# HarryL-Git/ampnet

Hardware: AMD Instinct MI355X
Metric: AMPConv edges/sec (fwd+bwd) (higher is better)
Workload: dtype f32

## Files before the change

### ampnet_amd/_lib.py

```python
import ctypes
import os

import torch

_HERE = os.path.dirname(os.path.abspath(__file__))
LIB_PATH = os.environ.get('AMPCONV_LIB_PATH', os.path.join(_HERE, 'libampconv.so'))

EXPECTED_ABI = 111

AMPCONV_F32 = 0
AMPCONV_BF16 = 1
DTYPES = {torch.float32: AMPCONV_F32, torch.bfloat16: AMPCONV_BF16}
PASS_FWD, PASS_DST, PASS_SRC = 0, 1, 2
FAMILY_BF16_MFMA, FAMILY_SMALL, FAMILY_MFMA, FAMILY_BLOCK, FAMILY_GENERIC = range(5)
HUB_CHUNK = int(os.environ.get('AMPCONV_HUB_CHUNK', 0))


def hub_chunk(num_edges):
    return HUB_CHUNK if HUB_CHUNK > 0 else (128 if num_edges >= (1 << 20) else 64)
COLSUM_BLOCKS = 1024


class View(ctypes.Structure):
    _fields_ = [('ptr', ctypes.c_void_p), ('node_stride', ctypes.c_int64),
# ... 90 lines not shown
    'ampconv_absmax': (_i32, [_vp, _i64, _i64, _i32, _i32, _vp, _i32, _vp]),
    'ampconv_planes_supported': (_i32, [_i32, _i32, _i32]),
    'ampconv_fwd_edge_planes': (_i32, [View, View, View, _vp, _vp, _i64, _i32, _i32, _i32, View, _vp, _i64, _vp, _vp, _vp]),
    'ampconv_bwd_edge_dst_planes': (_i32, [View, View, View, View, _vp, _vp, _i64, _i32, _i32, _i32, View, _vp, _i64, _vp,
                                           _vp, _vp, _vp, _vp, _vp]),
    'ampconv_bwd_edge_src_planes': (_i32, [View, View, View, View, _vp, _vp, _i64, _i32, _i32, _i32, View, View, _vp, _i64,
                                           _vp, _vp, _vp, _vp, _vp]),
    'ampconv_scaled_supported': (_i32, [_i32, _i32, _i32]),
    'ampconv_fwd_edge_scaled': (_i32, [View, View, View, _vp, _vp, _i64, _i32, _i32, _i32, View, _vp, _i64, _vp, _vp, _vp]),
    'ampconv_bwd_edge_dst_scaled': (_i32, [View, View, View, View, _vp, _vp, _i64, _i32, _i32, _i32, View, _vp, _i64, _vp,
                                           _vp, _vp, _vp, _vp, _vp]),
    'ampconv_bwd_edge_src_scaled': (_i32, [View, View, View, View, _vp, _vp, _vp, _i64, _i32, _i32, _i32, View, View, _vp,
                                           _i64, _vp, _vp, _vp, _vp, _vp]),
    'ampconv_token_supported': (_i32, [_i32, _i32, _i32, _i32]),
    'ampconv_fwd_edge_token': (_i32, [View, View, View, _vp, _vp, _i64, _i32, _i32, _i32, View, _vp, _i64, _vp, _i32, _vp]),
    'ampconv_bwd_edge_dst_token': (_i32, [View, View, View, View, _vp, _vp, _i64, _i32, _i32, _i32, View, _vp, _i64, _vp,
                                          _i32, _vp]),
    'ampconv_bwd_edge_src_token': (_i32, [View, View, View, View, _vp, _vp, _vp, _i64, _i32, _i32, _i32, View, View, _vp,
                                          _i64, _vp, _i32, _vp]),
    'ampconv_proj_out_bound': (_i32, [_vp, _i64, _i64, _i32, _i32, _vp, _vp, _vp, _vp]),
    'ampconv_proj_rows_planes': (_i32, [_vp, _i64, _i64, _i32, _vp, _i32, _vp, _vp, _i32, _i32, _vp, _i64, _vp, _vp, _vp,
                                        _i32, _i32, _vp]),
    'ampconv_planes_to_f32': (_i32, [_vp, _i64, _i64, _i32, _i32, _vp, _vp, _i64, _vp]),
    'ampconv_absmax_stats': (_i32, [_vp, _i64, _i64, _i32, _vp, _vp]),
    'ampconv_active_nodes_workspace_bytes': (_sz, [_i64]),
    'ampconv_active_nodes': (_i32, [_vp, _vp, _i64, _i32, _vp, _vp, _vp, _vp, _sz, _vp]),
    'ampconv_segment_mean': (_i32, [_vp, _vp, _vp, _i64, _i64, _vp, _vp]),
    'ampconv_mask_rows': (_i32, [_vp, _vp, _i64, _i64, _i32, _vp]),
    'ampconv_masked_colsum': (_i32, [_vp, _vp, _i64, _i32, _i32, _vp, _i32, _vp]),
    'ampconv_act_dropout_fwd': (_i32, [_vp, _i64, _i32, ctypes.c_uint64, ctypes.c_uint32, ctypes.c_float, _vp, _i32, _vp]),
    'ampconv_act_dropout_bwd': (_i32, [_vp, _vp, _i64, _i32, ctypes.c_uint64, ctypes.c_uint32, ctypes.c_float, _vp, _i32, _vp]),
    'ampconv_pool_fwd': (_i32, [_vp, _i64, _i32, _i32, _i32, _i32, ctypes.c_uint64, ctypes.c_uint32, ctypes.c_float, _vp, _i32,
                                _vp]),
    'ampconv_pool_bwd': (_i32, [_vp, _vp, _i64, _i32, _i32, _i32, _i32, ctypes.c_uint64, ctypes.c_uint32, ctypes.c_float, _vp,
                                _i32, _vp]),
    'ampconv_head_workspace_bytes': (_sz, [_i64, _i32, _i32]),
    'ampconv_head_fwd': (_i32, [_vp, _i64, _i32, _i64, _vp, _vp, _i32, _i32, _vp, _i32, _vp]),
    'ampconv_head_bwd': (_i32, [_vp, _i64, _i32, _i64, _vp, _i32, _i32, _vp, _vp, _vp, _vp, _vp, _vp, _sz, _i32, _vp]),
    'ampconv_head_nll_fwd': (_i32, [_vp, _i64, _i32, _i64, _vp, _vp, _i32, _vp, _vp, _vp, _i32, _i32, _vp, _vp, _vp, _vp,
                                    _i32, _vp]),
    'ampconv_head_nll_bwd': (_i32, [_vp, _i64, _i32, _i64, _vp, _vp, _i32, _vp, _vp, _vp, _i32, _i32, _vp, _vp, _vp, _vp,
                                    _vp, _sz, _i32, _vp]),
    'ampconv_norm_workspace_bytes': (_sz, [_i64, _i32]),
    'ampconv_norm_fwd': (_i32, [_vp, _i64, _i32, _vp, _vp, ctypes.c_float, _i32, ctypes.c_uint64, ctypes.c_uint32,
                                ctypes.c_float, _vp, _vp, _i32, _vp]),
    'ampconv_norm_bwd': (_i32, [_vp, _vp, _vp, _i64, _i32, _vp, _vp, _i32, ctypes.c_uint64, ctypes.c_uint32, ctypes.c_float,
# ... 75 lines not shown
```

### ampnet_amd/conv/functional.py

```python
import dataclasses
import os

import torch

from .. import _lib
from .._lib import ptr as _ptr
from ..graph import EdgeCSR, _stream
from .projection import (Projections, _aligned, _tn_matmul, gemm_precision, mask_rows, masked_colsum,
                         proj_image, proj_images, proj_native, proj_rows, proj_wgrad)


def _view(buf2d, col_off, L, dh):
    assert buf2d.is_contiguous() and buf2d.dtype in (torch.float32, torch.bfloat16)
    W = buf2d.size(1)
    return _lib.View(buf2d.data_ptr() + buf2d.element_size() * col_off, L * W, W, dh)


SOFTMAX_STATS = os.environ.get('AMPCONV_SOFTMAX_STATS', '1') != '0'
NODE_LISTS = os.environ.get('AMPCONV_NODE_LISTS', '1') != '0'
PROJ_SCALED = os.environ.get('AMPCONV_PROJ_SCALED', '1') != '0'
PROJ_SCALED_MIN_ELEMENTS = 1 << 24


EDGE_PLANES = os.environ.get('AMPCONV_EDGE_PLANES', '1') != '0'
# ... 8 lines not shown
        if (hit is not None and hit[0]() is key and hit[1] == key._version and hit[4] == (key.data_ptr(), tuple(key.shape))
                and hit[2].device == t2.device):
            return hit[2], hit[3]
    lib = _lib.load()
    t2 = _aligned(t2)
    st = torch.empty(2, dtype=torch.float32, device=t2.device)
    _lib.check(lib.ampconv_absmax_stats(t2.data_ptr(), t2.stride(0), t2.size(0), t2.size(1), st.data_ptr(), _stream()),
               'ampconv_absmax_stats')
    amax, smin = st.tolist()
    narrow = not (smin * float(1 << RANGE_LOG2) < amax)
    if key is not None:
        if len(_STATS_CACHE) >= 16:
            for k in [k for k, v in _STATS_CACHE.items() if v[0]() is None] or list(_STATS_CACHE)[:8]:
                _STATS_CACHE.pop(k, None)
        _STATS_CACHE[id(key)] = (weakref.ref(key), key._version, st, narrow, (key.data_ptr(), tuple(key.shape)))
    return st, narrow


def planes_to_f32(buf2d, bound, dh=32):
    out = torch.empty_like(buf2d)
    _lib.check(_lib.load().ampconv_planes_to_f32(buf2d.data_ptr(), buf2d.stride(0), buf2d.size(0), buf2d.size(1), dh,
                                                 bound.data_ptr(), out.data_ptr(), out.stride(0), _stream()),
               'ampconv_planes_to_f32')
    return out


def proj_out_bound(W, transpose, bias, amax, out):
    R, C = W.shape
    N, K = (C, R) if transpose else (R, C)
    sn, sk = (1, W.stride(0)) if transpose else (W.stride(0), 1)
    _lib.check(_lib.load().ampconv_proj_out_bound(W.data_ptr(), sn, sk, N, K, _ptr(bias), amax.data_ptr(), out.data_ptr(),
                                                  _stream()), 'ampconv_proj_out_bound')


def proj_rows_planes(a2, image, bound, bias=None, rowptr=None, L=0, row_scale=0, amax=None, out_amax=None, amax_col0=0,
                     dh=32):
    lib = _lib.load()
    img, N, K, wdt = image
    assert a2.dim() == 2 and a2.size(1) == K and a2.stride(1) == 1 and a2.dtype == wdt == torch.float32
    a2 = _aligned(a2)
    out = torch.empty(a2.size(0), N, dtype=wdt, device=a2.device)
    _lib.check(lib.ampconv_proj_rows_planes(a2.data_ptr(), a2.stride(0), a2.size(0), K, img.data_ptr(), N, _ptr(bias),
                                            _ptr(rowptr), L, row_scale, out.data_ptr(), out.stride(0), amax.data_ptr(),
                                            bound.data_ptr(), _ptr(out_amax), amax_col0, dh, _stream()),
               'ampconv_proj_rows_planes')
    return out
# ... 401 lines not shown
```

### ampnet_amd/csrc/edge_block_x3.hip

```cpp
#include "plane16.h"

namespace {
using namespace plane16;

constexpr int kRowB = 128;
constexpr int kTileRowsB = 16 * kRowB;

#define MFMA_X3(a, b, c) \
  __builtin_amdgcn_mfma_f32_16x16x32_bf16(__builtin_bit_cast(bf16x8, a), __builtin_bit_cast(bf16x8, b), (c), 0, 0, 0)
#define MFMA_XH(a, b, c) \
  __builtin_amdgcn_mfma_f32_16x16x32_f16(__builtin_bit_cast(f16x8, a), __builtin_bit_cast(f16x8, b), (c), 0, 0, 0)

template <int P>
struct XFrag {
  i32x4 p[P];
};

__device__ __forceinline__ float bfl(int u) { return __builtin_bit_cast(float, u << 16); }
__device__ __forceinline__ float bfh(int u) { return __builtin_bit_cast(float, u & (int)0xFFFF0000u); }

__device__ __forceinline__ int xoff(int j, int ch) { return j * kRowB + ((ch ^ (((j >> 1) & 3) << 1)) << 4); }

struct XArgs {
  ampconv_view_t Q, K, V, dO, O, dK, dV;
// ... 458 lines not shown
  __device__ __forceinline__ float dk_mul(const XArgs &a) const { return part_or(a, a.oscale); }
  __device__ __forceinline__ float dv_mul() const { return 1.f; }
};

template <int KS>
__device__ __forceinline__ float own_max_norm2(const XFrag<2> (&f)[KS]) {
  float q = frag_sumsq(f[0].p[0]);
  if constexpr (KS == 2) q += frag_sumsq(f[1].p[0]);
  const float t = groups_sum(q);
  return __builtin_bit_cast(float, __builtin_amdgcn_readfirstlane(__builtin_bit_cast(int, row16_max(t))));
}
__device__ __forceinline__ float ds_scale_x(float own2, float other) {
  return plane_scale(2.f * __builtin_sqrtf(own2) * (8.f * other));
}

struct FmtXH : Fp32Storage {
  static constexpr int kPlanes = 2;
  using Frag = XFrag<2>;
  static constexpr bool kQidx = false, kRecordMax = true, kSrcPairs = AMPCONV_XH_SRC_PAIRS;
  static constexpr float kPScale = 16384.f, kPUnscale = 1.f / 16384.f;
  static constexpr int fwd_mcb(int) { return AMPCONV_XH_FWD_MCB; }
  static constexpr int dst_mcb(int) { return AMPCONV_XH_DST_MCB; }

  static __device__ __forceinline__ void split(float x0, float x1, int (&w)[2]) { split2(x0, x1, w[0], w[1]); }
  static __device__ __forceinline__ f32x4 mma(const Frag &a, const Frag &b, f32x4 c) {
    c = MFMA_XH(a.p[1], b.p[0], c);
    c = MFMA_XH(a.p[0], b.p[1], c);
    return MFMA_XH(a.p[0], b.p[0], c);
  }

  float sq, uq, sg, ug;
  float sc;
  float sd, usd;
  __device__ __forceinline__ FmtXH(const XArgs &a, bool grad)
      : sq(plane_scale(a.bounds[0])), uq(1.f / sq), sg(grad ? plane_scale(a.bounds[1]) : 1.f), ug(1.f / sg),
        sc((a.qscale * uq) * uq), sd(1.f), usd(1.f) {}
  __device__ __forceinline__ float q_mul(const XArgs &) const { return sq; }
  __device__ __forceinline__ float g_mul(float inv) const { return inv * sg; }
  __device__ __forceinline__ float kv_mul() const { return sq; }
  template <int KS>
  __device__ __forceinline__ void dst_own(const Frag (&gf)[KS], const XArgs &a) {
    sd = ds_scale_x(own_max_norm2(gf), a.bounds[2] * sq);
    usd = 1.f / sd;
  }
  template <int KS>
  __device__ __forceinline__ void src_own(const Frag (&vf)[KS], const XArgs &a) {
    sd = ds_scale_x(own_max_norm2(vf), a.bounds[3] * sg);
// ... 627 lines not shown
```

### ampnet_amd/csrc/edge_mfma_bf16.hip

```cpp
#include "edge_wave16.h"

namespace {
using namespace wave16;

typedef unsigned short bf16_t;


#define MFMA_BF16(a, b, c) \
  __builtin_amdgcn_mfma_f32_16x16x32_bf16(__builtin_bit_cast(bf16x8, a), __builtin_bit_cast(bf16x8, b), (c), 0, 0, 0)

struct Args {
  ampconv_view_t Q, K, V, dO, O, dK, dV;
  const int32_t *ptr, *idx, *qidx;
  const float *cinv;
  HubArgs hub;
  int64_t n_units;
  int L, H;
  float qscale, oscale;
};

template <bool HALF>
__device__ __forceinline__ void store_tile(const ampconv_view_t &v, int64_t node, int h, const f32x4 (&T)[2][2],
                                           float scale, bool to_f32, int L, int lane) {
  const int g = lane >> 4;
// ... 4 lines not shown
#pragma unroll
      for (int mc = 0; mc < (HALF ? 1 : 2); ++mc) {
        const float a = T[mc][nt][0] * scale, b = T[mc][nt][1] * scale, c = T[mc][nt][2] * scale,
                    d = T[mc][nt][3] * scale;
        const int64_t off = node * v.node_stride + (int64_t)h * v.head_stride + (int64_t)i * v.row_stride +
                            4 * g + 16 * mc;
        if (to_f32)
          *reinterpret_cast<float4 *>(reinterpret_cast<float *>(v.ptr) + off) = make_float4(a, b, c, d);
        else
          *reinterpret_cast<i32x2 *>(reinterpret_cast<bf16_t *>(v.ptr) + off) =
              i32x2{cvt_pk_bf16(a, b), cvt_pk_bf16(c, d)};
      }
    }
  }
}

struct FmtB {
  using Args = ::Args;
  static constexpr int kPlanes = 1, kElemBytes = 2, kLoOff = 0, kTileBytes = kPlaneBytes;
  using Frag = wave16::Frag<1>;
  template <bool HALF> using Geom = PairGeom<4, 3, HALF ? 2 : 4, 1>;
  static constexpr bool kHalfZeroLds = false;
  template <bool HALF> static constexpr int mc_tiles() { return 2; }
  static constexpr bool kShadow = false;
  static constexpr float kMasked = kNegBig, kPMul = 1.f;

  static __device__ __forceinline__ f32x4 mma(const Frag &a, const Frag &b, f32x4 c) { return MFMA_BF16(a.p[0], b.p[0], c); }
  static __device__ __forceinline__ Frag cd_frag(const f32x4 &t0, const f32x4 &t1) {
    return Frag{{i32x4{cvt_pk_bf16(t0[0], t0[1]), cvt_pk_bf16(t0[2], t0[3]), cvt_pk_bf16(t1[0], t1[1]),
                       cvt_pk_bf16(t1[2], t1[3])}}};
  }

  struct Scales {
    float sc;
  };
  template <bool HALF> static __device__ __forceinline__ Scales scales(const Args &a) { return Scales{a.qscale}; }
  static __device__ __forceinline__ int64_t qrow(const Args &a, int64_t r) { return a.qidx ? uniform_ld(a.qidx + r) : r; }
  static __device__ __forceinline__ float fwd_scale(const Scales &, float mean) { return mean; }
  static __device__ __forceinline__ float ds_mul(const Args &, int deg, const Frag (&)[2]) {
    return deg > 0 ? 1.f / (float)deg : 0.f;
  }
  template <bool HALF> static __device__ __forceinline__ float dq_scale(const Args &a, const Scales &, float, bool hubp) {
    return hubp ? 1.f : a.oscale;
  }

  template <bool HALF>
  static __device__ __forceinline__ float store(const ampconv_view_t &v, int64_t node, int h, const f32x4 (&T)[2][2],
// ... 195 lines not shown
```

### ampnet_amd/csrc/edge_mfma_f16x2.hip

```cpp
#include "edge_wave16.h"

namespace {
using namespace wave16;

constexpr int kLoOff = kPlaneBytes + 64;
constexpr int kTileBytes = kLoOff + kPlaneBytes;
constexpr float kPScale = 16384.f;
constexpr float kPUnscale = 1.f / 16384.f;
constexpr float kSqrtDh = 5.656854249492381f;
constexpr float kMasked = -__builtin_inff();

#define MFMA_F16(a, b, c) \
  __builtin_amdgcn_mfma_f32_16x16x32_f16(__builtin_bit_cast(f16x8, a), __builtin_bit_cast(f16x8, b), (c), 0, 0, 0)

__device__ __forceinline__ f32x4 mfma3(const i32x4 &ah, const i32x4 &al, const i32x4 &bh, const i32x4 &bl, f32x4 c) {
  c = MFMA_F16(al, bh, c);
  c = MFMA_F16(ah, bl, c);
  return MFMA_F16(ah, bh, c);
}

__device__ __forceinline__ float tile_max_norm2(const i32x4 &f0, const i32x4 &f1) {
  const float t = fmaxf(groups_sum(frag_sumsq(f0)), groups_sum(frag_sumsq(f1)));
  return __builtin_bit_cast(float, __builtin_amdgcn_readfirstlane(__builtin_bit_cast(int, row16_max(t))));
}
__device__ __forceinline__ float ds_scale(float own2, float other) {
  return plane_scale(2.f * __builtin_sqrtf(own2) * (kSqrtDh * other));
}

__device__ __forceinline__ void cd_frag2(const f32x4 &t0, float t1_0, i32x4 &hi, i32x4 &lo) {
  int h0, l0, h1, l1, h2, l2;
  split2(t0[0], t0[1], h0, l0);
  split2(t0[2], t0[3], h1, l1);
  split2(t1_0, 0.f, h2, l2);
  hi = i32x4{h0, h1, h2, 0};
  lo = i32x4{l0, l1, l2, 0};
}

struct Args {
  ampconv_view_t Q, K, V, dO, O, dK, dV;
  const int32_t *ptr, *idx;
  const float *bounds;
  float *absmax;
  const int32_t *spos;
  float *stats;
  HubArgs hub;
  int64_t n_units;
  int L, H;
};

template <bool QUARTER, int MC>
__device__ __forceinline__ float store_tile(const ampconv_view_t &v, int64_t node, int h, const f32x4 (&T)[MC][2],
                                            float scale, int L, int lane) {
  const int g = lane >> 4, n = lane & 15;
  float m = 0.f;
#pragma unroll
// ... 7 lines not shown
        const int64_t off = node * v.node_stride + (int64_t)h * v.head_stride + (int64_t)i * v.row_stride + 4 * g + 16 * mc;
        *reinterpret_cast<float4 *>(reinterpret_cast<float *>(v.ptr) + off) = o;
        m = finite_abs_max(m, o);
      }
    }
  }
  return m;
}

struct FmtP {
  using Args = ::Args;
  static constexpr int kPlanes = 2, kElemBytes = 4, kLoOff = ::kLoOff, kTileBytes = ::kTileBytes;
  using Frag = wave16::Frag<2>;
  template <bool HALF> using Geom = PairGeom<HALF ? 4 : 8, HALF ? 3 : 5, HALF ? 4 : 8, 2, ::kLoOff>;
  static constexpr bool kHalfZeroLds = true;
  template <bool HALF> static constexpr int mc_tiles() { return HALF ? 1 : 2; }
  static constexpr bool kShadow = true;
  static constexpr float kMasked = ::kMasked, kPMul = kPScale;

  static __device__ __forceinline__ f32x4 mma(const Frag &a, const Frag &b, f32x4 c) { return mfma3(a.p[0], a.p[1], b.p[0], b.p[1], c); }
  static __device__ __forceinline__ Frag cd_frag(const f32x4 &t0, const f32x4 &t1) {
    Frag f;
    cd_frag2(t0, t1[0], f.p[0], f.p[1]);
    return f;
  }

  struct Scales {
    float uq, ug, sc;
  };
  template <bool HALF> static constexpr float inv_sqrt_dh() { return HALF ? 0.25f : 0.17677669529663687f; }
  template <bool HALF> static __device__ __forceinline__ Scales scales(const Args &a) {
    const float uq = 1.f / plane_scale(uniform_ld(a.bounds)), ug = 1.f / plane_scale(uniform_ld(a.bounds + 1));
    return Scales{uq, ug, (kLog2e * inv_sqrt_dh<HALF>() * uq) * uq};
  }
  static __device__ __forceinline__ int64_t qrow(const Args &, int64_t r) { return r; }
  static __device__ __forceinline__ float fwd_scale(const Scales &k, float mean) { return kPUnscale * k.uq * mean; }
  static __device__ __forceinline__ float ds_mul(const Args &a, int, const Frag (&gB)[2]) {
    return ds_scale(tile_max_norm2(gB[0].p[0], gB[1].p[0]), uniform_ld(a.bounds + 2) * plane_scale(uniform_ld(a.bounds)));
  }
  template <bool HALF> static __device__ __forceinline__ float dq_scale(const Args &, const Scales &k, float ss, bool hubp) {
    return (((1.f / ss) * k.uq) * k.ug) * k.uq * (hubp ? 1.f : inv_sqrt_dh<HALF>());
  }

  template <bool HALF>
  static __device__ __forceinline__ float store(const ampconv_view_t &v, int64_t node, int h, const f32x4 (&T)[HALF ? 1 : 2][2],
                                                float scale, bool, int L, int lane) {
// ... 261 lines not shown
```

### ampnet_amd/csrc/edge_wave16.h

```cpp
#pragma once
#include "plane16.h"

namespace wave16 {
using namespace plane16;

constexpr int kWavesPerBlock = 4;
constexpr int DH = 32;
constexpr int kRowBytes = DH * 2;
constexpr int kPlaneBytes = kLmax * kRowBytes;

template <int P>
struct Frag {
  i32x4 p[P];
};

struct Unit {
  int lane, wave;
  int64_t row, onode;
  int h, beg, end, deg;
};
template <class Fmt, bool HALF, class Body>
__device__ __forceinline__ void for_unit(const typename Fmt::Args &a, const ampconv_view_t &out0, const ampconv_view_t *out1,
                                         const Body &body) {
  Unit u;
// ... 74 lines not shown
  for (int pl = 0; pl < P; ++pl) f.p[pl] = i32x4{0, 0, 0, 0};
  if (j < L && (!HALF || kg < 2)) {
#pragma unroll
    for (int pl = P - 1; pl >= 0; --pl)
      f.p[pl] = *reinterpret_cast<const i32x4 *>(base + (unsigned)j * row_bytes + pl * (HALF ? kRowBytes / 2 : kRowBytes) + 16 * kg);
  }
  return f;
}
template <class Fmt>
__device__ __forceinline__ typename Fmt::Frag lds_rowfrag(const char *img, int mt, int lane) {
  typename Fmt::Frag f;
#pragma unroll
  for (int pl = 0; pl < Fmt::kPlanes; ++pl) f.p[pl] = rowfrag(img + pl * Fmt::kLoOff, mt, lane);
  return f;
}
template <class Fmt>
__device__ __forceinline__ typename Fmt::Frag lds_colfrag(const char *img, int mc, int lane) {
  typename Fmt::Frag f;
#pragma unroll
  for (int pl = 0; pl < Fmt::kPlanes; ++pl) f.p[pl] = colfrag(img + pl * Fmt::kLoOff, mc, lane);
  return f;
}

template <bool FULL>
__device__ __forceinline__ float column_softmax(f32x4 &t0, f32x4 &t1, float sc, float mul, float masked, int L, int g) {
  if (!FULL) {
#pragma unroll
    for (int q = 0; q < 4; ++q)
      if (4 * g + q >= L) t0[q] = masked;
    if (16 + g >= L) t1[0] = masked;
  }
  float m = fmaxf(fmaxf(fmaxf(t0[0], t0[1]), fmaxf(t0[2], t0[3])), t1[0]);
  m = groups_max(m);
#pragma unroll
  for (int q = 0; q < 4; ++q) t0[q] = fast_exp2((t0[q] - m) * sc);
  t1[0] = fast_exp2((t1[0] - m) * sc);
  float l = ((t0[0] + t0[1]) + (t0[2] + t0[3])) + t1[0];
  l = groups_sum(l);
  const float inv = fast_rcp(l) * mul;
#pragma unroll
  for (int q = 0; q < 4; ++q) t0[q] *= inv;
  t1[0] *= inv;
  t1[1] = t1[2] = t1[3] = 0.f;
  return fmaf(m, sc, __builtin_amdgcn_logf(l));
}

template <class Fmt, bool FULL, bool HALF>
__device__ __forceinline__ void fwd_body(const typename Fmt::Args &a) {
  using F = typename Fmt::Frag;
  using G = typename Fmt::template Geom<HALF>;
  constexpr int MC = Fmt::template mc_tiles<HALF>(), TB = Fmt::kTileBytes, EB = Fmt::kElemBytes;
  __shared__ __attribute__((aligned(16))) char lds_all[kWavesPerBlock][2 * TB];
  for_unit<Fmt, HALF>(a, a.O, nullptr, [&](const Unit &u) __attribute__((always_inline)) {
    const int lane = u.lane, h = u.h, beg = u.beg, end = u.end;
    const int L = a.L, g = lane >> 4;
    char *Kt = lds_all[u.wave], *Vt = Kt + TB;
    const typename Fmt::Scales k = Fmt::template scales<HALF>(a);

    F qB[2];
    {
      const char *qb = slot_ptr<EB>(a.Q, Fmt::qrow(a, u.row), h);
      const unsigned rb = (unsigned)a.Q.row_stride * EB;
#pragma unroll
      for (int nt = 0; nt < 2; ++nt) qB[nt] = frag_global<Fmt::kPlanes, HALF, false>(qb, rb, nt, L, lane);
    }
    if (!FULL || (HALF && Fmt::kHalfZeroLds)) lds_zero(Kt, 2 * TB, lane);
    f32x4 OT[MC][2];
#pragma unroll
    for (int mc = 0; mc < MC; ++mc) OT[mc][0] = OT[mc][1] = f32x4{0.f, 0.f, 0.f, 0.f};

    Pair16<G::NLD> kv;
    IdxWindow win;
    const unsigned krb = (unsigned)a.K.row_stride * EB, vrb = (unsigned)a.V.row_stride * EB;
    auto fetch = [&](int p) {
      const int64_t s = idxwin_get<false>(win, a.idx, nullptr, p, end, lane, nullptr);
      pair16_load<FULL, G>(kv, slot_ptr<EB>(a.K, s, h), krb, slot_ptr<EB>(a.V, s, h), vrb, L, lane);
    };
    if (beg < end) {
      idxwin_load<false>(win, a.idx, nullptr, beg, end, lane);
      fetch(beg);
    }
    for (int p = beg; p < end; ++p) {
      pair16_to_lds<FULL, G, TB>(Kt, kv, L, lane);
      if (p + 1 < end) fetch(p + 1);
      __builtin_amdgcn_wave_barrier();

      f32x4 S[2][2];
#pragma unroll
      for (int mt = 0; mt < 2; ++mt) {
        const F kA = lds_rowfrag<Fmt>(Kt, mt, lane);
#pragma unroll
        for (int nt = 0; nt < 2; ++nt) S[mt][nt] = Fmt::mma(kA, qB[nt], f32x4{0.f, 0.f, 0.f, 0.f});
      }
      F pB[2];
#pragma unroll
      for (int nt = 0; nt < 2; ++nt) {
        column_softmax<FULL>(S[0][nt], S[1][nt], k.sc, Fmt::kPMul, Fmt::kMasked, L, g);
        if (!Fmt::kShadow) pB[nt] = Fmt::cd_frag(S[0][nt], S[1][nt]);
      }
      F vA[MC];
      if (Fmt::kShadow) TR_PRE_READ();
#pragma unroll
      for (int mc = 0; mc < MC; ++mc) vA[mc] = lds_colfrag<Fmt>(Vt, mc, lane);
      if (Fmt::kShadow) {
#pragma unroll
        for (int nt = 0; nt < 2; ++nt) pB[nt] = Fmt::cd_frag(S[0][nt], S[1][nt]);
      }
      TR_FRAG_FENCE();
#pragma unroll
      for (int mc = 0; mc < MC; ++mc)
#pragma unroll
        for (int nt = 0; nt < 2; ++nt) OT[mc][nt] = Fmt::mma(vA[mc], pB[nt], OT[mc][nt]);
      __builtin_amdgcn_wave_barrier();
    }
    const bool hubp = a.hub.mode == 2;
    Fmt::template store<HALF>(a.O, u.onode, h, OT, Fmt::fwd_scale(k, hubp ? 1.f : (u.deg > 0 ? 1.f / (float)u.deg : 0.f)),
                              hubp, L, lane);
  });
}

template <class Fmt, bool FULL, bool STATS, bool HALF>
__device__ __forceinline__ void bwd_dst_body(const typename Fmt::Args &a) {
  using F = typename Fmt::Frag;
  using G = typename Fmt::template Geom<HALF>;
  constexpr int MC = Fmt::template mc_tiles<HALF>(), TB = Fmt::kTileBytes, EB = Fmt::kElemBytes;
  __shared__ __attribute__((aligned(16))) char lds_all[kWavesPerBlock][2 * TB];
  for_unit<Fmt, HALF>(a, a.O, nullptr, [&](const Unit &u) __attribute__((always_inline)) {
    const int lane = u.lane, h = u.h, beg = u.beg, end = u.end;
    const int L = a.L, g = lane >> 4;
// ... 29 lines not shown
    if (beg < end) {
      idxwin_load<STATS>(win, a.idx, sposf, beg, end, lane);
      fetch(beg);
    }
    for (int p = beg; p < end; ++p) {
      pair16_to_lds<FULL, G, TB>(Kt, kv, L, lane);
      cposf = cposf_next;
      if (p + 1 < end) fetch(p + 1);
      __builtin_amdgcn_wave_barrier();

      f32x4 S[2][2], dP[2][2];
      float lse[2], dlt[2];
#pragma unroll
      for (int mt = 0; mt < 2; ++mt) {
        const F kA = lds_rowfrag<Fmt>(Kt, mt, lane);
        const F vA = lds_rowfrag<Fmt>(Vt, mt, lane);
#pragma unroll
        for (int nt = 0; nt < 2; ++nt) {
          S[mt][nt] = Fmt::mma(kA, qB[nt], f32x4{0.f, 0.f, 0.f, 0.f});
          dP[mt][nt] = Fmt::mma(vA, gB[nt], f32x4{0.f, 0.f, 0.f, 0.f});
        }
      }
      F sB[2];
#pragma unroll
      for (int nt = 0; nt < 2; ++nt) {
        lse[nt] = column_softmax<FULL>(S[0][nt], S[1][nt], k.sc, 1.f, Fmt::kMasked, L, g);
        float part = S[1][nt][0] * dP[1][nt][0];
#pragma unroll
        for (int q = 0; q < 4; ++q) part = fmaf(S[0][nt][q], dP[0][nt][q], part);
        const float delta = groups_sum(part);
        dlt[nt] = delta;
#pragma unroll
        for (int q = 0; q < 4; ++q) S[0][nt][q] *= (dP[0][nt][q] - delta) * dsm;
        S[1][nt][0] *= (dP[1][nt][0] - delta) * dsm;
        if (!Fmt::kShadow) sB[nt] = Fmt::cd_frag(S[0][nt], S[1][nt]);
      }
      F kC[MC];
      if (Fmt::kShadow) TR_PRE_READ();
#pragma unroll
      for (int mc = 0; mc < MC; ++mc) kC[mc] = lds_colfrag<Fmt>(Kt, mc, lane);
      if (Fmt::kShadow) {
#pragma unroll
        for (int nt = 0; nt < 2; ++nt) sB[nt] = Fmt::cd_frag(S[0][nt], S[1][nt]);
      }
      TR_FRAG_FENCE();
#pragma unroll
      for (int mc = 0; mc < MC; ++mc)
#pragma unroll
        for (int nt = 0; nt < 2; ++nt) dQT[mc][nt] = Fmt::mma(kC[mc], sB[nt], dQT[mc][nt]);
      if constexpr (STATS) {
        float *st = a.stats + ((int64_t)__builtin_bit_cast(int, cposf) * a.H + h) * kStatsPerUnit;
        if (lane < L) {
          st[lane] = lane < 16 ? lse[0] : lse[1];
          st[kLmax + lane] = lane < 16 ? dlt[0] : dlt[1];
        }
      }
      __builtin_amdgcn_wave_barrier();
    }
    const bool hubp = a.hub.mode == 2;
    const float m = Fmt::template store<HALF>(a.O, u.onode, h, dQT, Fmt::template dq_scale<HALF>(a, k, dsm, hubp), hubp, L, lane);
    Fmt::record_absmax(a, m);
  });
}

#define WAVE16_KERNELS(K) {{K<false, false>, K<true, false>}, {K<false, true>, K<true, true>}}
#define WAVE16_KERNELS_STATS(K, S) {{K<false, S, false>, K<true, S, false>}, {K<false, S, true>, K<true, S, true>}}
// ... 7 lines not shown
```

### ampnet_amd/csrc/operand_scale.hip

```cpp
#include "proj_common.h"

using namespace proj;

namespace {
__global__ __launch_bounds__(1024) void out_bound_kernel(const float *__restrict__ W, int64_t sn, int64_t sk, int N, int K,
                                                         const float *__restrict__ bias, const float *__restrict__ amax,
                                                         float *__restrict__ out) {
  __shared__ float red[2][16];
  const int lane = threadIdx.x & 63, w = threadIdx.x >> 6;
  float l1 = 0.f, bm = 0.f;
  for (int n = w; n < N; n += 16) {
    float sum = 0.f;
    for (int k = lane; k < K; k += 64) sum += finite_abs(W[(int64_t)n * sn + (int64_t)k * sk]);
    l1 = fmaxf(l1, wave_sum(sum));
  }
  if (bias)
    for (int n = threadIdx.x; n < N; n += 1024) bm = fmaxf(bm, finite_abs(bias[n]));
  bm = wave_max(bm);
  if (lane == 0) { red[0][w] = l1; red[1][w] = bm; }
  __syncthreads();
  if (threadIdx.x == 0) {
    for (int i = 1; i < 16; ++i) { l1 = fmaxf(l1, red[0][i]); bm = fmaxf(bm, red[1][i]); }
    out[0] = *amax * l1 + bm;
  }
// ... 31 lines not shown
    float *o = out + row * ldo + slot * dh + 8 * c;
    *reinterpret_cast<float4 *>(o) = make_float4(v[0], v[1], v[2], v[3]);
    *reinterpret_cast<float4 *>(o + 4) = make_float4(v[4], v[5], v[6], v[7]);
  }
}
}

extern "C" int ampconv_planes_to_f32(const void *X, int64_t ld, int64_t M, int K, int plane_dh, const float *bound, void *out,
                                     int64_t ldo, void *stream) {
  if (M < 0 || K <= 0 || (plane_dh != 32 && plane_dh != 16) || K % plane_dh || ld < K || ldo < K || ld % 4 || ldo % 4 || !bound)
    return AMPCONV_E_BADARG;
  if (M == 0) return AMPCONV_OK;
  if (!X || !out || (uintptr_t)X % 16 || (uintptr_t)out % 16) return AMPCONV_E_BADARG;
  const int64_t pieces = M * (K / 8);
  int64_t grid = (pieces + 255) / 256;
  const int64_t cap = (int64_t)cu_count() * 16;
  if (grid > cap) grid = cap;
  planes_to_f32_kernel<<<(unsigned)grid, 256, 0, (hipStream_t)stream>>>((const char *)X, ld, M, K / 8, plane_dh, bound,
                                                                        (float *)out, ldo);
  return ampconv_launch_status();
}

namespace {
template <typename T>
__global__ __launch_bounds__(256) void absmax_kernel(const T *__restrict__ X, int64_t ld, int64_t M, int K4,
                                                     float *__restrict__ out) {
  constexpr int EPP = 16 / sizeof(T);
  const int64_t total = M * K4;
  float m = 0.f;
  for (int64_t i = (int64_t)blockIdx.x * 256 + threadIdx.x; i < total; i += (int64_t)gridDim.x * 256) {
    const int64_t row = i / K4;
    const int c = (int)(i - row * K4);
    const uint4 raw = *reinterpret_cast<const uint4 *>(X + row * ld + (int64_t)c * EPP);
    if constexpr (sizeof(T) == 4) {
      m = fmaxf(m, fmaxf(fmaxf(finite_abs(__builtin_bit_cast(float, raw.x)), finite_abs(__builtin_bit_cast(float, raw.y))),
                         fmaxf(finite_abs(__builtin_bit_cast(float, raw.z)), finite_abs(__builtin_bit_cast(float, raw.w)))));
    } else {
      const unsigned u[4] = {raw.x, raw.y, raw.z, raw.w};
#pragma unroll
      for (int k = 0; k < 4; ++k)
        m = fmaxf(m, fmaxf(finite_abs(lo_as_f32(u[k])), finite_abs(hi_as_f32(u[k]))));
    }
  }
  __shared__ float red[4];
#pragma unroll
  for (int o = 32; o > 0; o >>= 1) m = fmaxf(m, __shfl_xor(m, o));
// ... 90 lines not shown
```

### ampnet_amd/csrc/plane16.h

```cpp
#pragma once
#include "mfma_tile.h"

namespace plane16 {

typedef int i32x4 __attribute__((ext_vector_type(4)));
typedef int i32x2 __attribute__((ext_vector_type(2)));
typedef float f32x2 __attribute__((ext_vector_type(2)));
typedef short s16x4 __attribute__((ext_vector_type(4)));
typedef _Float16 f16x2 __attribute__((ext_vector_type(2)));
typedef _Float16 f16x8 __attribute__((ext_vector_type(8)));
typedef __bf16 bf16x2 __attribute__((ext_vector_type(2)));
typedef __bf16 bf16x8 __attribute__((ext_vector_type(8)));

constexpr float kLog2e = 1.4426950408889634f;

__device__ __forceinline__ int cvt_pk_bf16(float a, float b) {
  f32x2 v = {a, b};
  return __builtin_bit_cast(int, __builtin_convertvector(v, bf16x2));
}
__device__ __forceinline__ int cvt_pk_f16(float a, float b) {
  f32x2 v = {a, b};
  return __builtin_bit_cast(int, __builtin_convertvector(v, f16x2));
}

__device__ __forceinline__ float plane_scale(float bound) {
  int e = (int)((__builtin_bit_cast(unsigned, bound) >> 23) & 0xFFu);
  e = e < 15 ? 15 : (e > 254 ? 254 : e);
  return __builtin_bit_cast(float, (unsigned)(268 - e) << 23);
}
__device__ __forceinline__ float plane_unscale(float bound) { return 1.f / plane_scale(bound); }

__device__ __forceinline__ void split2(float x0, float x1, int &h, int &l) {
  h = cvt_pk_f16(x0, x1);
  const f16x2 hv = __builtin_bit_cast(f16x2, h);
  l = cvt_pk_f16(x0 - (float)hv[0], x1 - (float)hv[1]);
}

__device__ __forceinline__ float frag_sumsq(const i32x4 &f) {
  float s = 0.f;
#pragma unroll
  for (int k = 0; k < 4; ++k) {
    const f16x2 v = __builtin_bit_cast(f16x2, f[k]);
    s = __builtin_amdgcn_fdot2(v, v, s, false);
  }
  return s;
}

__device__ __forceinline__ i32x2 tr_half(const char *p) {
  return __builtin_bit_cast(i32x2, __builtin_amdgcn_ds_read_tr16_b64_v4i16((__attribute__((address_space(3))) s16x4 *)p));
}
__device__ __forceinline__ i32x4 tr_frag(const char *p0, const char *p1) {
  const i32x2 ai = tr_half(p0), bi = tr_half(p1);
  return i32x4{ai[0], ai[1], bi[0], bi[1]};
}

// ... 38 lines not shown
```

### ampnet_amd/csrc/proj_gemm.hip

```cpp
#include <type_traits>
#include "proj_common.h"

namespace {
using namespace proj;

template <bool HP>
struct Pl {
  static constexpr int NP = HP ? 2 : 3;
  static constexpr int NQ = HP ? 3 : 6;
  static constexpr int kTile = NP * kFrag;
};
__device__ constexpr int kPA[2][6] = {{2, 1, 0, 1, 0, 0}, {1, 0, 0, 0, 0, 0}};
__device__ constexpr int kPB[2][6] = {{0, 1, 2, 0, 1, 0}, {0, 1, 0, 0, 0, 0}};
template <bool HP>
__device__ __forceinline__ f32x16 mfma_p(const i32x4 &a, const i32x4 &b, const f32x16 &c) {
  if constexpr (HP) return MFMA32H(a, b, c);
  else return MFMA32(a, b, c);
}

struct Pair3 {
  int h1, h2, h3;
};
__device__ __forceinline__ Pair3 split_pair(float x0, float x1) {
  const unsigned a = (unsigned)cvt_pk_bf16(x0, x1);
// ... 334 lines not shown
        const int ohi = a.plane_dh == 32 ? 16 * pc : 64 * (pc >> 1) + 16 * (pc & 1), olo = ohi + 2 * a.plane_dh;
#pragma unroll
        for (int i = 0; i < MTW; ++i) {
          const int rl0 = (MTW * wm + i) * 32;
          float fl[16];
#pragma unroll
          for (int g = 0; g < 4; ++g) {
            const float4 f4 = *reinterpret_cast<const float4 *>(fl_t + rl0 + 4 * fh + 8 * g);
            fl[4 * g] = f4.x; fl[4 * g + 1] = f4.y; fl[4 * g + 2] = f4.z; fl[4 * g + 3] = f4.w;
          }
#pragma unroll
          for (int j = 0; j < NTW; ++j) {
            const int colt = cur.col0 + (NTW * wn + j) * 32;
            const float bjs = bj[j] * so;
#pragma unroll
            for (int e = 0; e < 16; ++e)
              stage[((e & 3) + 8 * (e >> 2) + 4 * fh) * 32 + (fr ^ (((e >> 1) & 1) << 2))] = (acc[i][j][e] * kso + bjs) * fl[e];
            const bool rec = a.out_amax && colt >= a.amax_col0;
#pragma unroll
            for (int g = 0; g < 2; ++g) {
              const int row = pr + 16 * g;
              const float4 v0 = *reinterpret_cast<const float4 *>(stage + row * 32 + 4 * ((2 * pc) ^ ps));
              const float4 v1 = *reinterpret_cast<const float4 *>(stage + row * 32 + 4 * ((2 * pc + 1) ^ ps));
              const Pair3 p0 = split_pair_h(v0.x, v0.y, 1.f), p1 = split_pair_h(v0.z, v0.w, 1.f);
              const Pair3 p2 = split_pair_h(v1.x, v1.y, 1.f), p3 = split_pair_h(v1.z, v1.w, 1.f);
              if ((!decltype(ragged)::value || cur.row0 + rl0 + row < a.M) && (!RAGGED || colt < a.N)) {
                char *o = reinterpret_cast<char *>(a.out + (cur.row0 + rl0 + row) * a.ldc + colt);
                *reinterpret_cast<i32x4 *>(o + ohi) = i32x4{p0.h1, p1.h1, p2.h1, p3.h1};
                *reinterpret_cast<i32x4 *>(o + olo) = i32x4{p0.h2, p1.h2, p2.h2, p3.h2};
                if (rec) omax = finite_abs_max(finite_abs_max(omax, v0), v1);
              }
            }
          }
        }
      };
      auto store_tile = [&](auto ragged) {
#pragma unroll
        for (int i = 0; i < MTW; ++i) {
          const int rl0 = (MTW * wm + i) * 32;
          float fl[16];
#pragma unroll
          for (int g = 0; g < 4; ++g) {
            const float4 f4 = *reinterpret_cast<const float4 *>(fl_t + rl0 + 4 * fh + 8 * g);
            fl[4 * g] = f4.x; fl[4 * g + 1] = f4.y; fl[4 * g + 2] = f4.z; fl[4 * g + 3] = f4.w;
          }
#pragma unroll
          for (int j = 0; j < NTW; ++j) {
            const int colt = cur.col0 + (NTW * wn + j) * 32;
#pragma unroll
            for (int e = 0; e < 16; ++e)
              stage[((e & 3) + 8 * (e >> 2) + 4 * fh) * 32 + fr] =
                  ((HP ? acc[i][j][e] * ua * uw : acc[i][j][e]) + bj[j]) * fl[e];
            float *o = a.out + (cur.row0 + rl0 + sr) * a.ldc + colt + 4 * sc4;
// ... 405 lines not shown
```

### include/ampconv.h

```cpp
#ifndef AMPCONV_H_
#define AMPCONV_H_

#include <stddef.h>
#include <stdint.h>

#ifdef __cplusplus
extern "C" {
#endif

#define AMPCONV_VERSION 111

enum {
  AMPCONV_OK = 0,
  AMPCONV_E_BADARG = -1,
  AMPCONV_E_DTYPE = -2,
  AMPCONV_E_WORKSPACE = -3
};

enum { AMPCONV_F32 = 0, AMPCONV_BF16 = 1 };

typedef struct {
  void *ptr;
  int64_t node_stride;
  int64_t row_stride;
// ... 151 lines not shown
  int N, K;
  void *image;
} ampconv_weight_image_t;
int ampconv_proj_weight_images(int count, const ampconv_weight_image_t *jobs, int dtype, void *stream);
int ampconv_proj_rows(const void *A, int64_t lda, int64_t M, int K, const void *wimage, int N,
                      const void *bias, const int32_t *rowptr, int L, void *out, int64_t ldc,
                      const int32_t *nodes, int64_t n_nodes, const float *a_absmax,
                      float *out_absmax, int dtype, void *stream);
size_t ampconv_proj_wgrad_workspace_bytes(int64_t M, int Na, int Nb, int dtype);
int ampconv_proj_wgrad(const void *A, int64_t lda, const void *B, int64_t ldb, int64_t M, int Na,
                       int Nb, const int32_t *rowptr, int L, void *dW, void *colsum,
                       void *workspace, size_t workspace_bytes, const int32_t *nodes, int64_t n_nodes,
                       const float *a_absmax, const float *b_absmax, int dtype, void *stream);
int ampconv_absmax(const void *X, int64_t ld, int64_t M, int K, int dtype, float *out, int reset,
                   void *stream);
int ampconv_proj_out_bound(const void *W, int64_t stride_n, int64_t stride_k, int N, int K,
                           const void *bias, const float *a_absmax, float *out, void *stream);
int ampconv_proj_rows_planes(const void *A, int64_t lda, int64_t M, int K, const void *wimage, int N,
                             const void *bias, const int32_t *rowptr, int L, int row_scale, void *out,
                             int64_t ldc, const float *a_absmax, const float *out_bound,
                             float *out_absmax, int absmax_col0, int plane_dh, void *stream);
int ampconv_planes_to_f32(const void *X, int64_t ld, int64_t M, int K, int plane_dh, const float *bound,
                          void *out, int64_t ldo, void *stream);
int ampconv_absmax_stats(const void *X, int64_t ld, int64_t M, int K, float *out, void *stream);

int ampconv_saint_random_walk(const int32_t *cscptr, const int32_t *crow, const int64_t *start,
                              int64_t B, int walk_length, uint64_t seed, int64_t *walks, void *stream);
size_t ampconv_saint_workspace_bytes(int64_t N);
int ampconv_saint_nodes(const int64_t *nodes, int64_t n, int64_t N, int32_t *mark, int32_t *relabel,
                        int64_t *node_idx, int32_t *n_sub, void *workspace, size_t workspace_bytes,
                        void *stream);
int ampconv_saint_count_edges(const int64_t *node_idx, int64_t n_sub, const int32_t *cscptr,
                              const int32_t *crow, const int32_t *mark, int32_t *cnt, int32_t *off,
                              int32_t *e_sub, void *workspace, size_t workspace_bytes, void *stream);
int ampconv_saint_count_edges_bounded(const int64_t *node_idx, int64_t n_bound, const int32_t *n_sub_dev,
                                      const int32_t *cscptr, const int32_t *crow, const int32_t *mark,
                                      int32_t *cnt, int32_t *off, int32_t *e_sub, void *workspace,
                                      size_t workspace_bytes, void *stream);
int ampconv_saint_fill_edges(const int64_t *node_idx, int64_t n_sub, const int32_t *cscptr,
                             const int32_t *crow, const int32_t *cperm, const int32_t *mark,
                             const int32_t *relabel, const int32_t *off, int64_t E_sub,
                             int64_t *edge_index, int64_t *edge_id, void *stream);
int ampconv_saint_add_counts(const int64_t *idx, int64_t n, float *count, void *stream);
int ampconv_saint_norms(const float *node_count, const float *edge_count, const int64_t *edge_src,
                        int64_t N, int64_t E, float num_samples, float *node_norm, float *edge_norm,
                        void *stream);
// ... 183 lines not shown
```

Baseline: 25.92 million.

## Fuse softmax normalization into f16 hi/lo split via mixed-precision FMA

Result: no change. 26.16 million, median of 6 (+0.9%).

```diff
diff --git a/ampnet_amd/_lib.py b/ampnet_amd/_lib.py
--- a/ampnet_amd/_lib.py
+++ b/ampnet_amd/_lib.py
@@ -136,6 +136,7 @@
     'ampconv_proj_rows_planes': (_i32, [_vp, _i64, _i64, _i32, _vp, _i32, _vp, _vp, _i32, _i32, _vp, _i64, _vp, _vp, _vp,
                                         _i32, _i32, _vp]),
     'ampconv_planes_to_f32': (_i32, [_vp, _i64, _i64, _i32, _i32, _vp, _vp, _i64, _vp]),
+    'ampconv_f32_to_planes': (_i32, [_vp, _i64, _i64, _i32, _i32, _vp, _vp, _i64, _vp]),
     'ampconv_absmax_stats': (_i32, [_vp, _i64, _i64, _i32, _vp, _vp]),
     'ampconv_active_nodes_workspace_bytes': (_sz, [_i64]),
     'ampconv_active_nodes': (_i32, [_vp, _vp, _i64, _i32, _vp, _vp, _vp, _vp, _sz, _vp]),
diff --git a/ampnet_amd/conv/functional.py b/ampnet_amd/conv/functional.py
--- a/ampnet_amd/conv/functional.py
+++ b/ampnet_amd/conv/functional.py
@@ -54,6 +54,14 @@
     _lib.check(_lib.load().ampconv_planes_to_f32(buf2d.data_ptr(), buf2d.stride(0), buf2d.size(0), buf2d.size(1), dh,
                                                  bound.data_ptr(), out.data_ptr(), out.stride(0), _stream()),
                'ampconv_planes_to_f32')
+    return out
+
+
+def f32_to_planes(x2d, bound, dh=32):
+    out = torch.empty_like(x2d)
+    _lib.check(_lib.load().ampconv_f32_to_planes(x2d.data_ptr(), x2d.stride(0), x2d.size(0), x2d.size(1), dh,
+                                                 bound.data_ptr(), out.data_ptr(), out.stride(0), _stream()),
+               'ampconv_f32_to_planes')
     return out
 
 
diff --git a/ampnet_amd/csrc/edge_block_x3.hip b/ampnet_amd/csrc/edge_block_x3.hip
--- a/ampnet_amd/csrc/edge_block_x3.hip
+++ b/ampnet_amd/csrc/edge_block_x3.hip
@@ -504,7 +504,7 @@
   static constexpr int fwd_mcb(int) { return AMPCONV_XH_FWD_MCB; }
   static constexpr int dst_mcb(int) { return AMPCONV_XH_DST_MCB; }
 
-  static __device__ __forceinline__ void split(float x0, float x1, int (&w)[2]) { split2(x0, x1, w[0], w[1]); }
+  static __device__ __forceinline__ void split(float x0, float x1, int (&w)[2]) { split2_c(x0, x1, w[0], w[1]); }
   static __device__ __forceinline__ f32x4 mma(const Frag &a, const Frag &b, f32x4 c) {
     c = MFMA_XH(a.p[1], b.p[0], c);
     c = MFMA_XH(a.p[0], b.p[1], c);
diff --git a/ampnet_amd/csrc/edge_mfma_bf16.hip b/ampnet_amd/csrc/edge_mfma_bf16.hip
--- a/ampnet_amd/csrc/edge_mfma_bf16.hip
+++ b/ampnet_amd/csrc/edge_mfma_bf16.hip
@@ -50,7 +50,7 @@
   template <bool HALF> using Geom = PairGeom<4, 3, HALF ? 2 : 4, 1>;
   static constexpr bool kHalfZeroLds = false;
   template <bool HALF> static constexpr int mc_tiles() { return 2; }
-  static constexpr bool kShadow = false;
+  static constexpr bool kShadow = false, kProdSplit = false;
   static constexpr float kMasked = kNegBig, kPMul = 1.f;
 
   static __device__ __forceinline__ f32x4 mma(const Frag &a, const Frag &b, f32x4 c) { return MFMA_BF16(a.p[0], b.p[0], c); }
diff --git a/ampnet_amd/csrc/edge_mfma_f16x2.hip b/ampnet_amd/csrc/edge_mfma_f16x2.hip
--- a/ampnet_amd/csrc/edge_mfma_f16x2.hip
+++ b/ampnet_amd/csrc/edge_mfma_f16x2.hip
@@ -31,6 +31,15 @@
   int h0, l0, h1, l1, h2, l2;
   split2(t0[0], t0[1], h0, l0);
   split2(t0[2], t0[3], h1, l1);
+  split2(t1_0, 0.f, h2, l2);
+  hi = i32x4{h0, h1, h2, 0};
+  lo = i32x4{l0, l1, l2, 0};
+}
+
+__device__ __forceinline__ void cd_frag2_prod(const f32x4 &a, const f32x4 &b, float t1_0, i32x4 &hi, i32x4 &lo) {
+  int h0, l0, h1, l1, h2, l2;
+  split2_prod(a[0], b[0], a[1], b[1], h0, l0);
+  split2_prod(a[2], b[2], a[3], b[3], h1, l1);
   split2(t1_0, 0.f, h2, l2);
   hi = i32x4{h0, h1, h2, 0};
   lo = i32x4{l0, l1, l2, 0};
@@ -84,6 +93,12 @@
   static __device__ __forceinline__ Frag cd_frag(const f32x4 &t0, const f32x4 &t1) {
     Frag f;
     cd_frag2(t0, t1[0], f.p[0], f.p[1]);
+    return f;
+  }
+  static constexpr bool kProdSplit = true;
+  static __device__ __forceinline__ Frag cd_frag_prod(const f32x4 &a, const f32x4 &b, const f32x4 &t1) {
+    Frag f;
+    cd_frag2_prod(a, b, t1[0], f.p[0], f.p[1]);
     return f;
   }
 
diff --git a/ampnet_amd/csrc/edge_wave16.h b/ampnet_amd/csrc/edge_wave16.h
--- a/ampnet_amd/csrc/edge_wave16.h
+++ b/ampnet_amd/csrc/edge_wave16.h
@@ -120,8 +120,9 @@
   return f;
 }
 
-template <bool FULL>
-__device__ __forceinline__ float column_softmax(f32x4 &t0, f32x4 &t1, float sc, float mul, float masked, int L, int g) {
+template <bool FULL, bool DEFER = false>
+__device__ __forceinline__ float column_softmax(f32x4 &t0, f32x4 &t1, float sc, float mul, float masked, int L, int g,
+                                                float *norm = nullptr) {
   if (!FULL) {
 #pragma unroll
     for (int q = 0; q < 4; ++q)
@@ -136,8 +137,12 @@
   float l = ((t0[0] + t0[1]) + (t0[2] + t0[3])) + t1[0];
   l = groups_sum(l);
   const float inv = fast_rcp(l) * mul;
-#pragma unroll
-  for (int q = 0; q < 4; ++q) t0[q] *= inv;
+  if (DEFER) {
+    *norm = inv;
+  } else {
+#pragma unroll
+    for (int q = 0; q < 4; ++q) t0[q] *= inv;
+  }
   t1[0] *= inv;
   t1[1] = t1[2] = t1[3] = 0.f;
   return fmaf(m, sc, __builtin_amdgcn_logf(l));
@@ -148,6 +153,7 @@
   using F = typename Fmt::Frag;
   using G = typename Fmt::template Geom<HALF>;
   constexpr int MC = Fmt::template mc_tiles<HALF>(), TB = Fmt::kTileBytes, EB = Fmt::kElemBytes;
+  static_assert(!Fmt::kProdSplit || Fmt::kShadow, "the product split sits in the shadow of the transposed reads");
   __shared__ __attribute__((aligned(16))) char lds_all[kWavesPerBlock][2 * TB];
   for_unit<Fmt, HALF>(a, a.O, nullptr, [&](const Unit &u) __attribute__((always_inline)) {
     const int lane = u.lane, h = u.h, beg = u.beg, end = u.end;
@@ -191,9 +197,10 @@
         for (int nt = 0; nt < 2; ++nt) S[mt][nt] = Fmt::mma(kA, qB[nt], f32x4{0.f, 0.f, 0.f, 0.f});
       }
       F pB[2];
+      float pn[2];
 #pragma unroll
       for (int nt = 0; nt < 2; ++nt) {
-        column_softmax<FULL>(S[0][nt], S[1][nt], k.sc, Fmt::kPMul, Fmt::kMasked, L, g);
+        column_softmax<FULL, Fmt::kProdSplit>(S[0][nt], S[1][nt], k.sc, Fmt::kPMul, Fmt::kMasked, L, g, &pn[nt]);
         if (!Fmt::kShadow) pB[nt] = Fmt::cd_frag(S[0][nt], S[1][nt]);
       }
       F vA[MC];
@@ -202,7 +209,10 @@
       for (int mc = 0; mc < MC; ++mc) vA[mc] = lds_colfrag<Fmt>(Vt, mc, lane);
       if (Fmt::kShadow) {
 #pragma unroll
-        for (int nt = 0; nt < 2; ++nt) pB[nt] = Fmt::cd_frag(S[0][nt], S[1][nt]);
+        for (int nt = 0; nt < 2; ++nt) {
+          if constexpr (Fmt::kProdSplit) pB[nt] = Fmt::cd_frag_prod(S[0][nt], f32x4{pn[nt], pn[nt], pn[nt], pn[nt]}, S[1][nt]);
+          else pB[nt] = Fmt::cd_frag(S[0][nt], S[1][nt]);
+        }
       }
       TR_FRAG_FENCE();
 #pragma unroll
@@ -278,6 +288,11 @@
         }
       }
       F sB[2];
+      constexpr bool kSplitNow = !Fmt::kShadow || (Fmt::kProdSplit && HALF);
+      auto split_ds = [&](int nt) __attribute__((always_inline)) {
+        if constexpr (Fmt::kProdSplit) return Fmt::cd_frag_prod(S[0][nt], dP[0][nt], S[1][nt]);
+        else return Fmt::cd_frag(S[0][nt], S[1][nt]);
+      };
 #pragma unroll
       for (int nt = 0; nt < 2; ++nt) {
         lse[nt] = column_softmax<FULL>(S[0][nt], S[1][nt], k.sc, 1.f, Fmt::kMasked, L, g);
@@ -286,18 +301,23 @@
         for (int q = 0; q < 4; ++q) part = fmaf(S[0][nt][q], dP[0][nt][q], part);
         const float delta = groups_sum(part);
         dlt[nt] = delta;
-#pragma unroll
-        for (int q = 0; q < 4; ++q) S[0][nt][q] *= (dP[0][nt][q] - delta) * dsm;
+        if constexpr (Fmt::kProdSplit) {
+#pragma unroll
+          for (int q = 0; q < 4; ++q) dP[0][nt][q] = (dP[0][nt][q] - delta) * dsm;
+        } else {
+#pragma unroll
+          for (int q = 0; q < 4; ++q) S[0][nt][q] *= (dP[0][nt][q] - delta) * dsm;
+        }
         S[1][nt][0] *= (dP[1][nt][0] - delta) * dsm;
-        if (!Fmt::kShadow) sB[nt] = Fmt::cd_frag(S[0][nt], S[1][nt]);
+        if (kSplitNow) sB[nt] = split_ds(nt);
       }
       F kC[MC];
       if (Fmt::kShadow) TR_PRE_READ();
 #pragma unroll
       for (int mc = 0; mc < MC; ++mc) kC[mc] = lds_colfrag<Fmt>(Kt, mc, lane);
-      if (Fmt::kShadow) {
-#pragma unroll
-        for (int nt = 0; nt < 2; ++nt) sB[nt] = Fmt::cd_frag(S[0][nt], S[1][nt]);
+      if (!kSplitNow) {
+#pragma unroll
+        for (int nt = 0; nt < 2; ++nt) sB[nt] = split_ds(nt);
       }
       TR_FRAG_FENCE();
 #pragma unroll
diff --git a/ampnet_amd/csrc/operand_scale.hip b/ampnet_amd/csrc/operand_scale.hip
--- a/ampnet_amd/csrc/operand_scale.hip
+++ b/ampnet_amd/csrc/operand_scale.hip
@@ -77,6 +77,44 @@
 }
 
 namespace {
+__global__ __launch_bounds__(256) void f32_to_planes_kernel(const float *__restrict__ X, int64_t ld, int64_t M, int K8, int dh,
+                                                            const float *__restrict__ bound, char *__restrict__ out,
+                                                            int64_t ldo) {
+  const float s = plane_scale(*bound);
+  const int pps = dh / 8;
+  const int64_t total = M * K8;
+  for (int64_t i = (int64_t)blockIdx.x * 256 + threadIdx.x; i < total; i += (int64_t)gridDim.x * 256) {
+    const int64_t row = i / K8;
+    const int r = (int)(i - row * K8), slot = r / pps, c = r - slot * pps;
+    const float *src = X + row * ld + slot * dh + 8 * c;
+    const float4 a = *reinterpret_cast<const float4 *>(src), b = *reinterpret_cast<const float4 *>(src + 4);
+    const float v[8] = {a.x, a.y, a.z, a.w, b.x, b.y, b.z, b.w};
+    int h[4], l[4];
+#pragma unroll
+    for (int k = 0; k < 4; ++k) split2(v[2 * k] * s, v[2 * k + 1] * s, h[k], l[k]);
+    char *dst = out + (row * ldo + (int64_t)slot * dh) * 4 + 16 * c;
+    *reinterpret_cast<i32x4 *>(dst) = i32x4{h[0], h[1], h[2], h[3]};
+    *reinterpret_cast<i32x4 *>(dst + 2 * dh) = i32x4{l[0], l[1], l[2], l[3]};
+  }
+}
+}
+
+extern "C" int ampconv_f32_to_planes(const void *X, int64_t ld, int64_t M, int K, int plane_dh, const float *bound, void *out,
+                                     int64_t ldo, void *stream) {
+  if (M < 0 || K <= 0 || (plane_dh != 32 && plane_dh != 16) || K % plane_dh || ld < K || ldo < K || ld % 4 || ldo % 4 || !bound)
+    return AMPCONV_E_BADARG;
+  if (M == 0) return AMPCONV_OK;
+  if (!X || !out || (uintptr_t)X % 16 || (uintptr_t)out % 16) return AMPCONV_E_BADARG;
+  const int64_t pieces = M * (K / 8);
+  int64_t grid = (pieces + 255) / 256;
+  const int64_t cap = (int64_t)cu_count() * 16;
+  if (grid > cap) grid = cap;
+  f32_to_planes_kernel<<<(unsigned)grid, 256, 0, (hipStream_t)stream>>>((const float *)X, ld, M, K / 8, plane_dh, bound,
+                                                                        (char *)out, ldo);
+  return ampconv_launch_status();
+}
+
+namespace {
 template <typename T>
 __global__ __launch_bounds__(256) void absmax_kernel(const T *__restrict__ X, int64_t ld, int64_t M, int K4,
                                                      float *__restrict__ out) {
diff --git a/ampnet_amd/csrc/plane16.h b/ampnet_amd/csrc/plane16.h
--- a/ampnet_amd/csrc/plane16.h
+++ b/ampnet_amd/csrc/plane16.h
@@ -31,6 +31,25 @@
 __device__ __forceinline__ float plane_unscale(float bound) { return 1.f / plane_scale(bound); }
 
 __device__ __forceinline__ void split2(float x0, float x1, int &h, int &l) {
+  h = cvt_pk_f16(x0, x1);
+  int lo;
+  if (__builtin_constant_p(x1) && x1 == 0.f) {
+    lo = 0;
+    asm("v_fma_mixlo_f16 %0, %1, -1.0, %2 op_sel_hi:[1,0,0]" : "+v"(lo) : "v"(h), "v"(x0));
+  } else {
+    asm("v_fma_mixlo_f16 %0, %1, -1.0, %2 op_sel_hi:[1,0,0]" : "=v"(lo) : "v"(h), "v"(x0));
+    asm("v_fma_mixhi_f16 %0, %1, -1.0, %2 op_sel:[1,0,0] op_sel_hi:[1,0,0]" : "+v"(lo) : "v"(h), "v"(x1));
+  }
+  l = lo;
+}
+__device__ __forceinline__ void split2_prod(float a0, float b0, float a1, float b1, int &h, int &l) {
+  h = cvt_pk_f16(a0 * b0, a1 * b1);
+  float r0, r1;
+  asm("v_fma_mix_f32 %0, %1, %2, -%3 op_sel_hi:[0,0,1]" : "=v"(r0) : "v"(a0), "v"(b0), "v"(h));
+  asm("v_fma_mix_f32 %0, %1, %2, -%3 op_sel:[0,0,1] op_sel_hi:[0,0,1]" : "=v"(r1) : "v"(a1), "v"(b1), "v"(h));
+  l = cvt_pk_f16(r0, r1);
+}
+__device__ __forceinline__ void split2_c(float x0, float x1, int &h, int &l) {
   h = cvt_pk_f16(x0, x1);
   const f16x2 hv = __builtin_bit_cast(f16x2, h);
   l = cvt_pk_f16(x0 - (float)hv[0], x1 - (float)hv[1]);
diff --git a/ampnet_amd/csrc/proj_gemm.hip b/ampnet_amd/csrc/proj_gemm.hip
--- a/ampnet_amd/csrc/proj_gemm.hip
+++ b/ampnet_amd/csrc/proj_gemm.hip
@@ -380,13 +380,14 @@
               const int row = pr + 16 * g;
               const float4 v0 = *reinterpret_cast<const float4 *>(stage + row * 32 + 4 * ((2 * pc) ^ ps));
               const float4 v1 = *reinterpret_cast<const float4 *>(stage + row * 32 + 4 * ((2 * pc + 1) ^ ps));
+              const bool live = (!decltype(ragged)::value || cur.row0 + rl0 + row < a.M) && (!RAGGED || colt < a.N);
+              if (live && rec) omax = finite_abs_max(finite_abs_max(omax, v0), v1);
               const Pair3 p0 = split_pair_h(v0.x, v0.y, 1.f), p1 = split_pair_h(v0.z, v0.w, 1.f);
               const Pair3 p2 = split_pair_h(v1.x, v1.y, 1.f), p3 = split_pair_h(v1.z, v1.w, 1.f);
-              if ((!decltype(ragged)::value || cur.row0 + rl0 + row < a.M) && (!RAGGED || colt < a.N)) {
+              if (live) {
                 char *o = reinterpret_cast<char *>(a.out + (cur.row0 + rl0 + row) * a.ldc + colt);
                 *reinterpret_cast<i32x4 *>(o + ohi) = i32x4{p0.h1, p1.h1, p2.h1, p3.h1};
                 *reinterpret_cast<i32x4 *>(o + olo) = i32x4{p0.h2, p1.h2, p2.h2, p3.h2};
-                if (rec) omax = finite_abs_max(finite_abs_max(omax, v0), v1);
               }
             }
           }
diff --git a/include/ampconv.h b/include/ampconv.h
--- a/include/ampconv.h
+++ b/include/ampconv.h
@@ -197,6 +197,8 @@
                              float *out_absmax, int absmax_col0, int plane_dh, void *stream);
 int ampconv_planes_to_f32(const void *X, int64_t ld, int64_t M, int K, int plane_dh, const float *bound,
                           void *out, int64_t ldo, void *stream);
+int ampconv_f32_to_planes(const void *X, int64_t ld, int64_t M, int K, int plane_dh, const float *bound,
+                          void *out, int64_t ldo, void *stream);
 int ampconv_absmax_stats(const void *X, int64_t ld, int64_t M, int K, float *out, void *stream);
 
 int ampconv_saint_random_walk(const int32_t *cscptr, const int32_t *crow, const int64_t *start,
```
